# BloodAxe/segmentation-networks-benchmark

Measured on AMD Instinct MI355X. Metric: images/sec/GPU (fwd+bwd) ZF_UNET 224x224 bs=32; 1/2/4/8-GPU scaling, higher is better.
Workload: dtype bf16; 1 GPU; ZF_UNET 224x224 bf16 bs=32/GPU, bce_dice, SGD lr 1e-3, Dropout2d 0.2, train step torch_train.py:180-190 (configs[1]); global_batch=32, parallelism=dp1

## Files before the change

### segmentation-networks-benchmark_amd/csrc/common.h

```cpp
#pragma once
#include <hip/hip_runtime.h>
#include <hip/hip_ext.h>
#include <limits.h>
#include <stdint.h>
#include <stdio.h>
#include <string.h>

#include "../../include/segnb_hip.h"

typedef __attribute__((ext_vector_type(8))) __bf16 bf16x8_t;
typedef __attribute__((ext_vector_type(16))) float f32x16_t;

struct bf16_t {
    unsigned short bits;
};

void segnb_set_error(const char* fmt, ...);

#define SEGNB_CHECK_ARG_AS(who, cond, msg)                           \
    do {                                                             \
        if (!(cond)) {                                               \
            segnb_set_error("%s: bad argument: %s", who, msg);       \
            return SEGNB_E_BADARG;                                   \
        }                                                            \
// ... 34 lines not shown
template <class T>
inline T segnb_plan_keep(T v) {
    static_assert(!(std::is_pointer<T>::value && std::is_class<typename std::remove_pointer<T>::type>::value),
                  "segnb_plan_keep: add an overload that copies this struct into the plan");
    return v;
}
inline const segnb_conv_geom* segnb_plan_keep(const segnb_conv_geom* g) {
    return g ? (const segnb_conv_geom*)segnb_plan_dup(g, sizeof(*g)) : g;
}
inline const segnb_loss_spec* segnb_plan_keep(const segnb_loss_spec* g) {
    return g ? (const segnb_loss_spec*)segnb_plan_dup(g, sizeof(*g)) : g;
}
inline const segnb_bn_reduce_epilogue* segnb_plan_keep(const segnb_bn_reduce_epilogue* g) {
    return g ? (const segnb_bn_reduce_epilogue*)segnb_plan_dup(g, sizeof(*g)) : g;
}
inline const segnb_bn_apply_epilogue* segnb_plan_keep(const segnb_bn_apply_epilogue* g) {
    return g ? (const segnb_bn_apply_epilogue*)segnb_plan_dup(g, sizeof(*g)) : g;
}
inline const segnb_upcat_src* segnb_plan_keep(const segnb_upcat_src* g) {
    return g ? (const segnb_upcat_src*)segnb_plan_dup(g, sizeof(*g)) : g;
}
inline const segnb_operand_tf* segnb_plan_keep(const segnb_operand_tf* g) {
    return g ? (const segnb_operand_tf*)segnb_plan_dup(g, sizeof(*g)) : g;
}
inline const segnb_wgrad_target* segnb_plan_keep(const segnb_wgrad_target* g) {
    return g ? (const segnb_wgrad_target*)segnb_plan_dup(g, sizeof(*g)) : g;
}
inline const segnb_act_epilogue* segnb_plan_keep(const segnb_act_epilogue* g) {
    return g ? (const segnb_act_epilogue*)segnb_plan_dup(g, sizeof(*g)) : g;
}
template <class... P, class... A>
inline void segnb_plan_record_call(const char* name, int (*fn)(P...), A... args) {
    static_assert(sizeof...(P) == sizeof...(A), "argument count");
    std::tuple<P...> kept(segnb_plan_keep((P)args)...);
    segnb_plan_push([fn, kept]() { return std::apply(fn, kept); }, name);
}
extern int g_segnb_census_on;
void segnb_census(const char* name);
#define SEGNB_PLAN_RECORD(fn, ...)                                                           \
    SegnbPlanScope plan_scope__;                                                             \
    if (plan_scope__.top && g_segnb_census_on) segnb_census(#fn);                            \
    if (plan_scope__.top && segnb_plan_recording()) segnb_plan_record_call(#fn, fn, __VA_ARGS__)
void segnb_plan_refuse(const char* why);
#define SEGNB_PLAN_REFUSE(why)                                         \
    SegnbPlanScope plan_scope__;                                       \
    if (plan_scope__.top && g_segnb_census_on) segnb_census(__func__); \
    if (plan_scope__.top && segnb_plan_recording()) segnb_plan_refuse(why)

int segnb_num_cus();
bool segnb_fprop_general_forced();
int segnb_knob_fprop_dma();
int segnb_knob_fprop_dma_cfg();
int segnb_knob_fprop_dma_dbg();
int segnb_knob_fprop_nostats();
int segnb_knob_rw_store_waves();
int segnb_knob_bnreduce_fused();
int segnb_knob_fprop_deepk();
int segnb_knob_fprop_thin();
enum segnb_try_outcome {
    SEGNB_TRY_DECLINED = 0,
    SEGNB_TRY_LAUNCHED,
    SEGNB_TRY_DELIVERED,
};
constexpr int SEGNB_LAUNCH_DECLINED = INT_MIN;
inline int segnb_try_launched(segnb_try_outcome* did, int rc) {
    if (rc == SEGNB_LAUNCH_DECLINED) {
        *did = SEGNB_TRY_DECLINED;
        return 0;
    }
    if (rc == 0) *did = SEGNB_TRY_LAUNCHED;
    return rc;
}
#define SEGNB_HOST_INLINE static inline __attribute__((always_inline))
template <class... K>
int segnb_opt_in_lds(const char* who, int bytes, K... kernels) {
    hipError_t e = hipSuccess;
    (void)(... && ((e = hipFuncSetAttribute(reinterpret_cast<const void*>(kernels), hipFuncAttributeMaxDynamicSharedMemorySize,
                                            bytes)) == hipSuccess));
    if (e != hipSuccess) segnb_set_error("%s hipFuncSetAttribute(%d bytes): %s", who, bytes, hipGetErrorString(e));
    return (int)e;
}
SEGNB_HOST_INLINE long long segnb_nhwc_bytes(long long npix, int ld, int C, int esz) { return ((npix - 1) * ld + C) * esz; }
SEGNB_HOST_INLINE bool segnb_fits_desc(long long bytes, unsigned* out = nullptr) {
    if (out != nullptr) *out = (unsigned)bytes;
    return bytes < (1ll << 31);
}
inline void segnb_kernel_took(segnb_try_outcome did, const char** served, const char* name) {
    if (did != SEGNB_TRY_DECLINED && *served == nullptr) *served = name;
}
template <class Args>
__attribute__((always_inline)) inline bool take_bn_reduce(Args& a, const segnb_conv_geom* g, const segnb_bn_reduce_epilogue* bn) {
    const long long yb = segnb_nhwc_bytes((long long)g->N * g->Ho * g->Wo, bn->ld_y, g->Co, 2);
    if (!segnb_fits_desc(yb)) return false;
    a.bn_y = (const bf16_t*)bn->y;
    a.bn_y_bytes = (unsigned)yb;
    a.bn_ld = bn->ld_y;
    a.bn_coef = bn->coef;
    a.bn_sums = bn->sums;
    a.bn_act = bn->act;
    a.bn_slope = bn->slope;
    return true;
}
template <class Args>
__attribute__((always_inline)) inline void take_act_epilogue(Args& a, const segnb_act_epilogue* ep) {
    a.ep_act = ep != nullptr ? ep->act : -1;
    a.ep_coef = ep != nullptr ? ep->coef : nullptr;
// ... 221 lines not shown
```

### segmentation-networks-benchmark_amd/csrc/fprop_dma.hip

```cpp
#include "common.h"

#include "fprop_dma.h"

#include <mutex>
#include <vector>

#ifndef SEGNB_EXP
#define SEGNB_EXP 0
#endif

namespace {

__device__ unsigned long long g_stamps[3 * 256 * 4];
#define FD_STAMP(role, step, k)                                                                      \
    do {                                                                                            \
        if (DBG && ((a.dbg & 32) || ((a.dbg & 64) && (role) == 0 && (k) == 0)) && blockIdx.x == 0 && lane == 0 &&  \
            (step) < 256)                                                                            \
            g_stamps[((role) * 256 + (step)) * 4 + (k)] = __builtin_amdgcn_s_memtime();             \
    } while (0)

template <int BN_, int R_, int WT_, int CW_M_, bool TALL_ = false, bool MF16_ = true, int NTAP_ = 9, int UP_ = 0>
struct WsCfg {
    static constexpr bool UPD_ = UP_ == 1;
    static constexpr bool UPF = UP_ == 2;
    static_assert(UP_ == 0 || (NTAP_ == 4 && !TALL_ && MF16_), "up-sampled segment forms: 2 x 2 window, 16x16x32 form");
    static constexpr int BN = BN_, R = R_, WT = WT_;
    static constexpr int NTAP = NTAP_, KW = NTAP_ == 9 ? 3 : 2, KH = KW;
    static constexpr bool UPD = UPD_;
    static constexpr int UP = UP_;
    static constexpr int NPL = UPD_ ? 4 : 1;
    static_assert(NTAP_ == 9 || NTAP_ == 4, "3 x 3 or 2 x 2 tap window");
    static_assert(!UPD_ || (NTAP_ == 4 && !TALL_ && MF16_), "plane gather: 2 x 2 window, 16x16x32 form");
    static constexpr bool TALL = TALL_;
    static constexpr bool MF16 = MF16_;
    static constexpr int BM = TALL_ ? 256 : (R_ * WT_ + 16 * CW_M_ - 1) / (16 * CW_M_) * (16 * CW_M_);
    static constexpr int TM16 = BM / CW_M_ / 16, TN16 = BN_ / (4 / CW_M_) / 16;
    static constexpr int NB = 4;
    static constexpr int NT = 512, NCW = 4, NLW = 4;
    static_assert(R * WT <= BM, "tile pixels");
    static constexpr int NRD = TM16 + TN16, NMF = TM16 * TN16;
    static constexpr int rd_before(int q) { return (q * NRD + NMF - 1) / NMF; }
    static constexpr int WAVES_M = CW_M_, WAVES_N = NCW / CW_M_;
    static constexpr int WM = BM / WAVES_M, WN = BN / WAVES_N;
    static constexpr int TM = WM / 32, TN = WN / 32;
    static constexpr int XR = R + KH - 1, XC = WT + 2, NPIX = XR * XC;
    static constexpr int APIECES = (NPIX + 7) / 8;
    static constexpr int A_BYTES = APIECES * 1024;
    static constexpr int NBW = 2, NAW = 2;
    static constexpr int APW = (APIECES + NAW - 1) / NAW;
    static constexpr int A_STEPS = NTAP - 2;
    static constexpr int APS = (APW + A_STEPS - 1) / A_STEPS;
    static constexpr int BPIECES = BN / 8;
    static constexpr int B_STAGE = BN * 128;
    static constexpr int BPW = BPIECES / NBW;
    static constexpr int OUT_ROW = BN * 2 + 16;
    static constexpr int OC = BN / 8;
    static constexpr int MT = NCW * 64;
    static constexpr int RPT = BM / (MT / OC);
    static constexpr int OFF_B = 2 * A_BYTES;
    static constexpr int OFF_STG = OFF_B + NB * B_STAGE;
    static constexpr int OFF_DUMMY = OFF_STG + BM * OUT_ROW;
    static constexpr int OFF_PIX = OFF_DUMMY + 1024;
    static constexpr int OFF_BIAS = OFF_PIX + 4 * BM * 4;
    static constexpr int OFF_SCALE = OFF_BIAS + BN * 4;
    static constexpr int OFF_TICKET = OFF_SCALE + BN * 4;
    static constexpr int SMEM = OFF_TICKET + 16;
    static constexpr int RED_BYTES = MT * 16 * 8;
    static_assert(WM % (MF16_ ? 16 : 32) == 0 && WN % (MF16_ ? 16 : 32) == 0 && WAVES_M * WAVES_N == NCW, "wave tiling");
    static_assert(BPIECES % NBW == 0 && NBW + NAW == NLW, "fetch wave roles");
    static_assert(MT % OC == 0 && MT >= 2 * BN && RPT <= 8 && BM <= MT && BM % (MT / OC) == 0, "store pass / statistics threads");
    static constexpr bool MASK_OK = MF16_ && !TALL_ && BM == 256 && CW_M_ == 4 && SMEM + 2048 <= 160 * 1024;
    static_assert(RED_BYTES <= OFF_STG, "statistics reduction scratch");
    static_assert(SMEM <= 160 * 1024, "LDS");
    static_assert(TM + TN <= 6, "fragment wait statement");
};

template <class C, bool DBG, bool EP = false, bool STATS = true, bool SPLITK = false, bool MASK = false>
__global__ __launch_bounds__(512) void conv_fprop_ws_kernel(const FdArgs a) {
    static_assert(!SPLITK || (!EP && !DBG && C::UP == 0 && C::NTAP == 9), "split K: plain 3 x 3 forward / data gradient");
    static_assert(!MASK || (STATS && !EP && !DBG && !SPLITK && C::MF16 && C::UP == 0 && C::NTAP == 9 && !C::TALL && C::BM == 256 &&
                            C::BN == 64 && C::WAVES_M == 4 && C::SMEM + 2048 <= 160 * 1024),
                  "activation mask: plain 3 x 3 data gradient, 16x16x32 form, 256 x 64 tiles, 2 KB of mask bytes behind the LDS layout");
    constexpr int BN = C::BN, R = C::R, WT = C::WT, BM = C::BM, TM = C::TM, TN = C::TN, XC = C::XC;
    constexpr int NT = C::NT, NB = C::NB, APW = C::APW, APS = C::APS, BPW = C::BPW, OC = C::OC, NLW = C::NLW;
    constexpr int OUT_ROW = C::OUT_ROW, NF = TM + TN;
    constexpr int NTAP = C::NTAP, KW = C::KW;
    constexpr int SM = NTAP & 3;

    extern __shared__ __attribute__((aligned(1024))) unsigned char smem[];
    int* sPix = reinterpret_cast<int*>(smem + C::OFF_PIX);
    float* sBias = reinterpret_cast<float*>(smem + C::OFF_BIAS);
    const unsigned lds0 = (unsigned)(size_t)smem;

    const int tid = threadIdx.x, lane = tid & 63, wave = __builtin_amdgcn_readfirstlane(tid >> 6);
    const int r = lane & 31, h = lane >> 5;
    const bool loader = wave >= C::NCW;
    const int lw = wave - C::NCW;
    const int wm = (wave & 3) / C::WAVES_N, wn = (wave & 3) % C::WAVES_N;

    int L_ = xcd_remap(blockIdx.x, gridDim.x);
    int ks_ = 0, nt_, gq_;
    if (C::TALL && a.ntmajor) {
        gq_ = L_ % a.GM;
        L_ /= a.GM;
        if constexpr (SPLITK) {
            ks_ = L_ % a.KS;
            L_ /= a.KS;
        }
        nt_ = L_;
    } else {
        if constexpr (SPLITK) {
            ks_ = L_ % a.KS;
            L_ /= a.KS;
        }
        nt_ = L_ % a.NTL;
        gq_ = L_ / a.NTL;
    }
    const int ks = ks_;
    const int c_off = SPLITK ? ks * a.NCH : 0;
    const int nt = nt_, gq = gq_;
    int n_base_ = nt * BN, w_row0_ = nt * BN, py_ = 0, px_ = 0;
    if constexpr (C::UPF) {
        const int ph = nt / a.NTLR, ct = nt - ph * a.NTLR;
        n_base_ = ct * BN;
        w_row0_ = ph * a.CoW + ct * BN;
        py_ = ph >> 1;
        px_ = ph & 1;
    }
    const int n_base = n_base_, w_row0 = w_row0_, py = py_, px = px_;

    const i32x4_t rs_x = make_rsrc4(a.x, a.x_bytes);
    const i32x4_t rs_w = make_rsrc4(a.w, a.w_bytes);
    const i32x4_t rs_u = make_rsrc4(a.u != nullptr ? a.u : a.x, a.u != nullptr ? a.u_bytes : a.x_bytes);

    float* sScale = reinterpret_cast<float*>(smem + C::OFF_SCALE);
    for (int c = tid; c < BN; c += NT) {
        const int co = n_base + c;
        const float bv = (a.bias != nullptr && co < a.bias_n) ? a.bias[co] : 0.f;
        float sc = 1.f, sh = bv;
        if constexpr (EP) {
// ... 437 lines not shown
        auto ks_combine = [&](auto&& get, auto&& set) {
            unsigned base = slab0;
            asm volatile("" : "+v"(base));
            if (a.KS == 2) {
                const unsigned other = base + (unsigned)(ks ^ 1) * 65536u;
                static_for<2>([&](auto h_c) {
                    constexpr int h8 = decltype(h_c)::value * 8;
                    f32x4_t o[8];
                    static_for<8>([&](auto q_c) { constexpr int q = decltype(q_c)::value; o[q] = ks_load(other + (h8 + q) * 1024u); });
                    static_for<8>([&](auto q_c) {
                        constexpr int q = decltype(q_c)::value;
                        set(std::integral_constant<int, h8 + q>{}, get(std::integral_constant<int, h8 + q>{}) + o[q]);
                    });
                    asm volatile("s_waitcnt vmcnt(0)" ::: "memory");
                });
            } else {
                static_for<4>([&](auto h_c) {
                    constexpr int h8 = decltype(h_c)::value * 4;
                    f32x4_t v[4][4];
                    static_for<4>([&](auto q_c) {
                        constexpr int q = decltype(q_c)::value;
#pragma unroll
                        for (int k = 0; k < 4; ++k)
                            v[q][k] = ks_load(k != ks ? base + (unsigned)k * 65536u + (h8 + q) * 1024u : OOB);
                    });
                    static_for<4>([&](auto q_c) {
                        constexpr int q = decltype(q_c)::value;
                        const f32x4_t own = get(std::integral_constant<int, h8 + q>{});
#pragma unroll
                        for (int k = 0; k < 4; ++k) v[q][k] = k == ks ? own : v[q][k];
                        set(std::integral_constant<int, h8 + q>{}, (v[q][0] + v[q][1]) + (v[q][2] + v[q][3]));
                    });
                    asm volatile("s_waitcnt vmcnt(0)" ::: "memory");
                });
            }
        };
        if constexpr (MF16) {
            static_assert((TM16 == 4 && TN16 == 4) || (TM16 == 7 && TN16 == 2), "16x16x32 wave tile: 64 x 64 or 112 pixels x 32 channels");
            constexpr int NRD = C::NRD;
            static_assert(NRD + TM16 - 1 <= 15, "counted lgkmcnt");
            bf16x8_t fw[2][TN16], fx[2][TM16];
            auto issue = [&](int q, int set, int wbase, int xbase, int t, int k) {
                if (q == 0) { const int ad = a_rd16[t % KW][0][k] + xbase; FD_READ(fx[set][0], ad); }
                else if (q <= TN16) { const int ad = b_rd16[k][q - 1] + wbase; FD_READ(fw[set][q - 1], ad); }
                else { const int ad = a_rd16[t % KW][q - TN16][k] + xbase; FD_READ(fx[set][q - TN16], ad); }
            };
            int arow[KW];
#pragma unroll
            for (int k = 0; k < KW; ++k) arow[k] = __builtin_amdgcn_readfirstlane(a.dh[KW * k] * XC * 128);
            if (!(DBG && (a.dbg & 4))) {
#pragma unroll
                for (int q = 0; q < NRD; ++q) issue(q, 0, 0, arow[0], 0, 0);
            }
            int tile_no = 0;
            bool pending = false;
            for (; it < a.IT; it += a.GM, ++tile_no) {
                f32x4_t acc[TM16][TN16];
                uint2 prev[C::UPF ? TM16 : 1][C::UPF ? TN16 : 1];
                if constexpr (C::UPF) {
                    const int r16 = lane & 15, g4 = lane >> 4;
                    const int* tab = sPix + (tile_no & 3) * BM;
#pragma unroll
                    for (int i = 0; i < TM16; ++i) {
                        const int opix = tab[wm * C::WM + 16 * i + r16];
#pragma unroll
                        for (int j = 0; j < TN16; ++j) {
                            const int ch = n_base + wn * C::WN + 16 * j + 4 * g4;
                            uint2 v = make_uint2(0u, 0u);
                            if (opix >= 0 && ch < a.Co && !a.no_prev)
                                v = *reinterpret_cast<const uint2*>(a.out + (long long)opix * a.ld_out + ch);
                            prev[i][j] = v;
                        }
                    }
                }
                for (int c = 0; c < a.NCH; ++c, ++cg) {
                    const int a_base = (cg & 1) * C::A_BYTES;
                    const bool drain = pending && c == 0;
                    static_for<NTAP>([&](auto t_c) {
                        constexpr int t = decltype(t_c)::value;
                        constexpr int tn = t == NTAP - 1 ? 0 : t + 1;
                        auto& accr = acc;
                        const int bstage = ((cg * SM + t) & (NB - 1)) * C::B_STAGE;
                        const int bnext = ((cg * SM + t + 1) & (NB - 1)) * C::B_STAGE;
                        const int anext = t == NTAP - 1 ? ((cg + 1) & 1) * C::A_BYTES : a_base;
                        if (wave == 0) FD_STAMP(0, cg * 9 + t, 0);
                        constexpr bool row_tap9 = NTAP == 9 && t >= 1 && t <= C::RPT;
                        bool do_row = false;
                        int krow = t - 1;
                        if constexpr (NTAP == 9) {
                            do_row = drain;
                        } else {
                            const int si = c * NTAP + t;
                            krow = (si - 1) * a.RPS;
                            do_row = pending && si >= 1 && krow < C::RPT;
                        }
                        if constexpr (row_tap9 || NTAP != 9)
                            if (do_row) {
                                row_load(krow, sPix + ((tile_no + 3) & 3) * BM);
                                if constexpr (NTAP != 9)
                                    if (a.RPS == 2) row_load2(krow + 1, sPix + ((tile_no + 3) & 3) * BM);
                            }
                        if (!(SEGNB_EXP & 4) && !(DBG && (a.dbg & 4))) {
                            __builtin_amdgcn_s_setprio(1);
#pragma unroll
                            for (int kk = 0; kk < 2; ++kk) {
                                const int cur = kk, nxt = kk ^ 1;
                                const int wbase = kk == 0 ? bstage : bnext;
                                const int xbase = kk == 0 ? a_base + arow[t / KW] : anext + arow[tn / KW];
// ... 45 lines not shown
                    ks_last = ks_publish([&](auto p_c) { constexpr int p = decltype(p_c)::value; return acc[p / TN16][p % TN16]; });
                    if (ks_last)
                        ks_combine([&](auto p_c) { constexpr int p = decltype(p_c)::value; return acc[p / TN16][p % TN16]; },
                                   [&](auto p_c, const f32x4_t v) { constexpr int p = decltype(p_c)::value; acc[p / TN16][p % TN16] = v; });
                }
                if (!SPLITK || ks_last) {
                const int r16 = lane & 15, g4 = lane >> 4;
                float4 bv[TN16], sv[TN16];
                uint2 mrow[MASK ? TM16 : 1];
                if constexpr (MASK) {
#pragma unroll
                    for (int i = 0; i < TM16; ++i)
                        mrow[i] = *reinterpret_cast<const uint2*>(smem + C::SMEM + (wm * C::WM + 16 * i + r16) * 8);
                }
#pragma unroll
                for (int j = 0; j < TN16; ++j) {
                    if constexpr (!MASK) bv[j] = *reinterpret_cast<const float4*>(sBias + wn * C::WN + 16 * j + 4 * g4);
                    if constexpr (EP) sv[j] = *reinterpret_cast<const float4*>(sScale + wn * C::WN + 16 * j + 4 * g4);
                    else sv[j] = make_float4(1.f, 1.f, 1.f, 1.f);
                }
#pragma unroll
                for (int i = 0; i < TM16; ++i) {
                    const int row = wm * C::WM + 16 * i + r16;
#pragma unroll
                    for (int j = 0; j < TN16; ++j) {
                        const int col = wn * C::WN + 16 * j + 4 * g4;
                        uint2 pk;
                        if constexpr (C::UPF) {
                            const uint2 pv = prev[i][j];
                            const float v0 = acc[i][j][0] + __uint_as_float(pv.x << 16) + bv[j].x;
                            const float v1 = acc[i][j][1] + __uint_as_float(pv.x & 0xffff0000u) + bv[j].y;
                            const float v2 = acc[i][j][2] + __uint_as_float(pv.y << 16) + bv[j].z;
                            const float v3 = acc[i][j][3] + __uint_as_float(pv.y & 0xffff0000u) + bv[j].w;
                            pk.x = pack2bf(fmaxf(v0, v0 * upf_neg), fmaxf(v1, v1 * upf_neg));
                            pk.y = pack2bf(fmaxf(v2, v2 * upf_neg), fmaxf(v3, v3 * upf_neg));
                        } else if constexpr (MASK) {
                            const unsigned mb = (j < 2 ? mrow[i].x : mrow[i].y) >> (8 * ((2 * j + (g4 >> 1)) & 3) + 4 * (g4 & 1));
                            const unsigned g01 = pack2bf(acc[i][j][0], acc[i][j][1]);
                            const unsigned g23 = pack2bf(acc[i][j][2], acc[i][j][3]);
                            const float g0 = __uint_as_float(g01 << 16), g1 = __uint_as_float(g01 & 0xffff0000u);
                            const float g2 = __uint_as_float(g23 << 16), g3 = __uint_as_float(g23 & 0xffff0000u);
                            pk.x = pack2bf((mb & 1u) ? g0 : g0 * mask_neg, (mb & 2u) ? g1 : g1 * mask_neg);
                            pk.y = pack2bf((mb & 4u) ? g2 : g2 * mask_neg, (mb & 8u) ? g3 : g3 * mask_neg);
                        } else {
                        pk.x = pack2bf(ep(acc[i][j][0], sv[j].x, bv[j].x), ep(acc[i][j][1], sv[j].y, bv[j].y));
                        pk.y = pack2bf(ep(acc[i][j][2], sv[j].z, bv[j].z), ep(acc[i][j][3], sv[j].w, bv[j].w));
                        }
                        *reinterpret_cast<uint2*>(sOut + row * OUT_ROW + col * 2) = pk;
                    }
                }
                }
                pending = !SPLITK || ks_last;
            }
            tile_no_out = tile_no;
            pending_out = pending;
        } else {
            static_assert(MF16 || NTAP == 9, "the 32x32x16 form serves the 3 x 3 window only (fragment sets cycle with 36 slices)");

            bf16x8_t fr[3][NF];
            if (!(DBG && (a.dbg & 4))) {
    #pragma unroll
                for (int kk = 0; kk < 2; ++kk) {
    #pragma unroll
                    for (int j = 0; j < TN; ++j) {
                        const int ad = b_rd[j] ^ (kk << 5);
                        FD_READ(fr[kk][j], ad);
                    }
    #pragma unroll
                    for (int i = 0; i < TM; ++i) {
                        const int ad = a_rd[0][i] ^ (kk << 5);
                        FD_READ(fr[kk][TN + i], ad);
                    }
                }
            }
            int tile_no = 0;
            bool pending = false;
            for (; it < a.IT; it += a.GM, ++tile_no) {
                f32x16_t acc[TM][TN];
                for (int c = 0; c < a.NCH; ++c, ++cg) {
                    const int a_base = (cg & 1) * C::A_BYTES;
                    const bool drain = pending && c == 0;
                    static_for<9>([&](auto t_c) {
                        constexpr int t = decltype(t_c)::value;
                        constexpr int tn = t == 8 ? 0 : t + 1;
                        auto& accr = acc;
                        const int bstage = ((cg + t) & (NB - 1)) * C::B_STAGE;
                        const int bnext = ((cg + t + 1) & (NB - 1)) * C::B_STAGE;
                        const int anext = t == 8 ? ((cg + 1) & 1) * C::A_BYTES : a_base;
                        if (wave == 0) FD_STAMP(0, cg * 9 + t, 0);
                        constexpr bool row_tap = t >= 1 && t <= C::RPT;
                        if constexpr (row_tap)
                            if (drain) row_load(t - 1, sPix + ((tile_no + 3) & 3) * BM);
                        if (!(SEGNB_EXP & 4) && !(DBG && (a.dbg & 4))) {
                            __builtin_amdgcn_s_setprio(1);
    #pragma unroll
                            for (int kk = 0; kk < 4; ++kk) {
                                const int set_cur = (4 * t + kk) % 3, set_new = (4 * t + kk + 2) % 3;
                                int ad[NF];
                                if (kk < 2) {
    #pragma unroll
                                    for (int j = 0; j < TN; ++j) ad[j] = (b_rd[j] + bstage) ^ ((kk + 2) << 5);
    #pragma unroll
                                    for (int i = 0; i < TM; ++i) ad[TN + i] = (a_rd[t][i] + a_base) ^ ((kk + 2) << 5);
                                } else {
    #pragma unroll
                                    for (int j = 0; j < TN; ++j) ad[j] = (b_rd[j] + bnext) ^ ((kk - 2) << 5);
// ... 121 lines not shown
    static std::mutex mu;
    static std::vector<Ent> ents;
    int dev = 0;
    if (hipGetDevice(&dev) != hipSuccess) return -1;
    std::lock_guard<std::mutex> lock(mu);
    Ent* e = nullptr;
    for (auto& it : ents)
        if (it.dev == dev && it.stream == stream) e = &it;
    const bool grow = e == nullptr || slab_bytes > e->cap || ntiles > e->ncnt;
    if (grow) {
        hipStreamCaptureStatus cs = hipStreamCaptureStatusNone;
        if (hipStreamIsCapturing(stream, &cs) != hipSuccess || cs != hipStreamCaptureStatusNone) return -1;
        if (e == nullptr) {
            ents.push_back(Ent{dev, stream, nullptr, 0, nullptr, 0});
            e = &ents.back();
        }
        if (slab_bytes > e->cap) {
            float* p = nullptr;
            if (hipMalloc(&p, slab_bytes) != hipSuccess) return -1;
            e->slab = p;
            e->cap = slab_bytes;
        }
        if (ntiles > e->ncnt) {
            const int want = ntiles < 1024 ? 1024 : ntiles;
            int* c = nullptr;
            if (hipMalloc(&c, (size_t)want * sizeof(int)) != hipSuccess) return -1;
            if (hipMemsetAsync(c, 0, (size_t)want * sizeof(int), stream) != hipSuccess) return -1;
            e->cnt = c;
            e->ncnt = want;
        }
    }
    *slab = e->slab;
    *cnt = e->cnt;
    return 0;
}

template <class C>
int ksplit_factor(const FdArgs& a, int it_total, int ntl, int nch) {
    if (!C::TALL || !segnb_knob_fprop_ksplit()) return 1;
    if (a.ep_act >= 0 || a.dbg || a.up_out != nullptr) return 1;
    const long long tiles = (long long)it_total * ntl;
    int cus = segnb_knob_conv_cus();
    if (a.stats == nullptr) cus /= 2;
    int ks = 1;
    if (tiles * 2 <= cus && nch % 2 == 0 && nch / 2 >= 2) ks = 2;
    if (tiles * 4 <= cus && nch % 4 == 0 && nch / 4 >= 2) ks = 4;
    const int forced = segnb_knob_fprop_ksplit();
    if (forced > 1 && nch % forced == 0 && nch / forced >= 2 && (forced == 2 || forced == 4)) ks = forced;
    if (tiles * ks * 65536ll >= (1ll << 31)) return 1;
    return ks;
}

template <class C>
int launch_ws(FdArgs& a, hipStream_t stream) {
    if (a.bn_y != nullptr && !C::MASK_OK) return SEGNB_LAUNCH_DECLINED;
    static const int attr_rc = [] {
        int rc = segnb_opt_in_lds("fprop_ws", C::SMEM, conv_fprop_ws_kernel<C, false>, conv_fprop_ws_kernel<C, true>,
                                  conv_fprop_ws_kernel<C, false, true, false>, conv_fprop_ws_kernel<C, false, false, false>);
        if constexpr (C::MASK_OK) {
            if (rc == 0) rc = segnb_opt_in_lds("fprop_ws", C::SMEM + 2048, conv_fprop_ws_kernel<C, false, false, true, false, true>);
        }
        if constexpr (C::TALL) {
            if (rc == 0)
                rc = segnb_opt_in_lds("fprop_ws", C::SMEM, conv_fprop_ws_kernel<C, false, false, true, true>,
                                      conv_fprop_ws_kernel<C, false, false, false, true>);
        }
        return rc;
    }();
    if (attr_rc) return attr_rc;
    a.HB = (a.H + C::R - 1) / C::R;
    a.WB = (a.W + C::WT - 1) / C::WT;
    a.IT = a.N * a.HB * a.WB;
    if (C::TALL) {
        if (a.W > C::WT || a.Hi != a.H || a.Wi != a.W) return SEGNB_LAUNCH_DECLINED;
        a.IT = (a.N * (a.H + 1) + C::R - 1) / C::R;
    }
    a.NTL = (a.Co + C::BN - 1) / C::BN;
    a.NCH = a.Ci / 64;
    a.KS = 1;
    a.ntmajor = C::TALL ? 1 : 0;
    if constexpr (C::TALL) {
        const int ks = ksplit_factor<C>(a, a.IT, a.NTL, a.NCH);
        if (ks > 1 && ksplit_workspace(stream, (size_t)a.IT * a.NTL * ks * 65536, a.IT * a.NTL, &a.ks_slab, &a.ks_cnt) == 0) {
            a.KS = ks;
            a.NCH /= ks;
            a.GM = a.IT;
            a.ks_slab_bytes = (unsigned)((size_t)a.IT * a.NTL * ks * 65536);
            const dim3 grid(a.IT * a.NTL * ks);
            if (a.stats != nullptr || !segnb_knob_fprop_nostats())
                hipLaunchKernelGGL((conv_fprop_ws_kernel<C, false, false, true, true>), grid, dim3(C::NT), C::SMEM, stream, a);
            else
                hipLaunchKernelGGL((conv_fprop_ws_kernel<C, false, false, false, true>), grid, dim3(C::NT), C::SMEM, stream, a);
            return 0;
        }
    }
    int gm = segnb_knob_conv_cus() / a.NTL;
    if (gm < 1) gm = 1;
    if (gm > a.IT) gm = a.IT;
    a.GM = gm;
    if (a.bn_y != nullptr) {
        if constexpr (C::MASK_OK) {
            hipLaunchKernelGGL((conv_fprop_ws_kernel<C, false, false, true, false, true>), dim3(a.GM * a.NTL), dim3(C::NT), C::SMEM + 2048,
                               stream, a);
            return 0;
        } else {
            return SEGNB_LAUNCH_DECLINED;
        }
    }
    if (a.ep_act >= 0)
        hipLaunchKernelGGL((conv_fprop_ws_kernel<C, false, true, false>), dim3(a.GM * a.NTL), dim3(C::NT), C::SMEM, stream, a);
    else if (a.stats == nullptr && !a.dbg && segnb_knob_fprop_nostats())
        hipLaunchKernelGGL((conv_fprop_ws_kernel<C, false, false, false>), dim3(a.GM * a.NTL), dim3(C::NT), C::SMEM, stream, a);
    else if (a.dbg)
        hipLaunchKernelGGL((conv_fprop_ws_kernel<C, true>), dim3(a.GM * a.NTL), dim3(C::NT), C::SMEM, stream, a);
    else
        hipLaunchKernelGGL((conv_fprop_ws_kernel<C, false>), dim3(a.GM * a.NTL), dim3(C::NT), C::SMEM, stream, a);
    return 0;
}

using WsCfg14 = WsCfg<64, 14, 14, 2, false, true>;

bool ws14_serves(const FdArgs& a) {
    return a.H % 14 == 0 && a.W % 14 == 0 && a.W <= 56 && a.Co > 32 && a.bn_y == nullptr && a.ep_act < 0 && !a.dbg &&
           a.up_out == nullptr && segnb_knob_fprop_mf16();
}

int launch_ws14(FdArgs& a, hipStream_t stream) {
    using C = WsCfg14;
    static const int attr_rc = segnb_opt_in_lds("fprop_ws", C::SMEM, conv_fprop_ws_kernel<C, false>, conv_fprop_ws_kernel<C, false, false, false>);
    if (attr_rc) return attr_rc;
    a.HB = a.H / C::R;
    a.WB = a.W / C::WT;
    a.IT = a.N * a.HB * a.WB;
    a.NTL = (a.Co + C::BN - 1) / C::BN;
    a.NCH = a.Ci / 64;
    a.KS = 1;
    a.ntmajor = 0;
    int gm = segnb_knob_conv_cus() / a.NTL;
    if (gm < 1) gm = 1;
    if (gm > a.IT) gm = a.IT;
    a.GM = gm;
    if (g_segnb_census_on) segnb_census("tile:ws14");
    if (a.stats == nullptr && segnb_knob_fprop_nostats())
        hipLaunchKernelGGL((conv_fprop_ws_kernel<C, false, false, false>), dim3(a.GM * a.NTL), dim3(C::NT), C::SMEM, stream, a);
    else
        hipLaunchKernelGGL((conv_fprop_ws_kernel<C, false>), dim3(a.GM * a.NTL), dim3(C::NT), C::SMEM, stream, a);
    return 0;
}

template <class C>
int launch_ws_upd(FdArgs& a, hipStream_t stream) {
    static const int attr_rc = segnb_opt_in_lds("fprop_ws", C::SMEM, conv_fprop_ws_kernel<C, false, false, false>);
    if (attr_rc) return attr_rc;
    a.HB = (a.H + C::R - 1) / C::R;
    a.WB = (a.W + C::WT - 1) / C::WT;
    a.IT = a.N * a.HB * a.WB;
    a.NTL = (a.Co + C::BN - 1) / C::BN;
    a.P32 = a.Ci == 32;
    a.NCHP = a.P32 ? 1 : a.Ci / 64;
    a.NCH = a.P32 ? 2 : 4 * a.NCHP;
    a.RPS = a.NCH * C::NTAP - 1 < C::RPT ? 2 : 1;
    if ((a.NCH * C::NTAP - 1) * a.RPS < C::RPT) return SEGNB_LAUNCH_DECLINED;
    int gm = segnb_knob_conv_cus() / a.NTL;
    if (gm < 1) gm = 1;
    if (gm > a.IT) gm = a.IT;
    a.GM = gm;
    hipLaunchKernelGGL((conv_fprop_ws_kernel<C, false, false, false>), dim3(a.GM * a.NTL), dim3(C::NT), C::SMEM, stream, a);
    return 0;
}

template <class C>
int launch_ws_upf(FdArgs& a, hipStream_t stream) {
    static const int attr_rc = segnb_opt_in_lds("fprop_ws", C::SMEM, conv_fprop_ws_kernel<C, false, false, true>);
    if (attr_rc) return attr_rc;
    a.HB = (a.H + C::R - 1) / C::R;
    a.WB = (a.W + C::WT - 1) / C::WT;
    a.IT = a.N * a.HB * a.WB;
    a.NTLR = (a.Co + C::BN - 1) / C::BN;
    a.NTL = 4 * a.NTLR;
    a.NCH = a.Ci / 64;
    a.NCHP = a.NCH;
    a.P32 = 0;
    a.RPS = a.NCH * C::NTAP - 1 < C::RPT ? 2 : 1;
    if ((a.NCH * C::NTAP - 1) * a.RPS < C::RPT) return SEGNB_LAUNCH_DECLINED;
    int gm = segnb_knob_conv_cus() / a.NTL;
    if (gm < 1) gm = 1;
    if (gm > a.IT) gm = a.IT;
    a.GM = gm;
    hipLaunchKernelGGL((conv_fprop_ws_kernel<C, false, false, true>), dim3(a.GM * a.NTL), dim3(C::NT), C::SMEM, stream, a);
    return 0;
}

bool upd_geometry(const segnb_conv_geom* g) {
    if (g->ntaps != 16 || g->in_step != 2 || !whole_output(g) || g->Hi != 2 * g->Ho || g->Wi != 2 * g->Wo) return false;
    if ((g->Ci % 64 != 0 && g->Ci != 32) || g->Co <= 32 || g->Wo < 12) return false;
// ... 215 lines not shown
```

### segmentation-networks-benchmark_amd/csrc/runtime.hip

```cpp
#include <stdarg.h>
#include <stdlib.h>

#include "common.h"

static thread_local char g_err[512] = "";

void segnb_set_error(const char* fmt, ...) {
    va_list ap;
    va_start(ap, fmt);
    vsnprintf(g_err, sizeof(g_err), fmt, ap);
    va_end(ap);
}

int segnb_num_cus() {
    static int cus = 0;
    if (cus > 0) return cus;
    int dev = 0;
    hipDeviceProp_t prop;
    if (hipGetDevice(&dev) != hipSuccess || hipGetDeviceProperties(&prop, dev) != hipSuccess) return 256;
    cus = prop.multiProcessorCount > 0 ? prop.multiProcessorCount : 256;
    return cus;
}

extern "C" const char* segnb_last_error(void) { return g_err; }
// ... 258 lines not shown
int segnb_knob_fprop_mf16() {
    if (g_fprop_mf16 == -2) {
        const char* e = getenv("SEGNB_FPROP_MF16");
        g_fprop_mf16 = (e != nullptr && e[0] == '0') ? 0 : 1;
    }
    return g_fprop_mf16;
}
static int g_fprop_upd = -2;
int segnb_knob_fprop_upd() {
    if (g_fprop_upd == -2) {
        const char* e = getenv("SEGNB_FPROP_UPD");
        g_fprop_upd = (e != nullptr && e[0] == '0') ? 0 : 1;
    }
    return g_fprop_upd;
}
static int g_fprop_mask = -2;
int segnb_knob_fprop_mask() {
    if (g_fprop_mask == -2) {
        const char* e = getenv("SEGNB_FPROP_MASK");
        g_fprop_mask = (e != nullptr && e[0] == '0') ? 0 : 1;
    }
    return g_fprop_mask;
}
static int g_fprop_drop = -2;
int segnb_knob_fprop_drop() {
    if (g_fprop_drop == -2) {
        const char* e = getenv("SEGNB_FPROP_DROP");
        g_fprop_drop = (e != nullptr && e[0] == '0') ? 0 : 1;
    }
    return g_fprop_drop;
}
static int g_fprop_nostats = 1;
int segnb_knob_fprop_nostats() { return g_fprop_nostats; }
static int g_rw_store_waves = 4;
int segnb_knob_rw_store_waves() { return g_rw_store_waves; }
static int g_bnreduce_fused = -2;
int segnb_knob_bnreduce_fused() {
    if (g_bnreduce_fused == -2) {
        const char* e = getenv("SEGNB_BNREDUCE_FUSED");
        g_bnreduce_fused = (e != nullptr && e[0] == '0') ? 0 : 1;
    }
    return g_bnreduce_fused;
}
static int g_fprop_ksplit = -2;
int segnb_knob_fprop_ksplit() {
    if (g_fprop_ksplit == -2) {
        const char* e = getenv("SEGNB_FPROP_KSPLIT");
        g_fprop_ksplit = e != nullptr ? atoi(e) : 1;
    }
    return g_fprop_ksplit;
}
static int g_fprop_dma_dbg = 0;
int segnb_knob_fprop_dma_dbg() { return g_fprop_dma_dbg; }
extern "C" int segnb_wg_cu_share(int pct) {
    SEGNB_PLAN_RECORD(segnb_wg_cu_share, pct);
    g_wg_cu_pct = pct < 0 ? 0 : (pct > 100 ? 100 : pct);
    return 0;
}

static thread_local segnb_wgrad_target g_wg_target;
static thread_local bool g_wg_target_armed = false;
extern "C" int segnb_wgrad_target_arm(const segnb_wgrad_target* t) {
    SEGNB_PLAN_RECORD(segnb_wgrad_target_arm, t);
    SEGNB_CHECK_ARG(t != nullptr && t->gw != nullptr, "NULL target");
    SEGNB_CHECK_ARG(t->ntaps >= 1 && t->ntaps <= SEGNB_MAX_TAPS && t->Ci > 0 && t->Co > 0 && t->s_in >= t->ntaps && t->ci_off >= 0 &&
                        t->s_out >= (long long)(t->ci_off + t->Ci) * t->s_in, "bad target layout");
    for (int i = 0; i < t->ntaps; ++i) SEGNB_CHECK_ARG(t->kpos[i] >= 0 && t->kpos[i] < t->s_in, "bad kernel position");
    g_wg_target = *t;
    g_wg_target_armed = true;
    return 0;
}
const segnb_wgrad_target* segnb_take_wgrad_target() {
    if (!g_wg_target_armed) return nullptr;
    g_wg_target_armed = false;
    return &g_wg_target;
}

extern "C" int segnb_tune(const char* key, int value) {
    SEGNB_PLAN_REFUSE("segnb_tune inside a recorded plan");
    SEGNB_CHECK_ARG(key != nullptr, "NULL key");
    if (strcmp(key, "fprop_dma") == 0) {
        g_fprop_dma = value ? 1 : 0;
        return 0;
    }
    if (strcmp(key, "fprop_dma_cfg") == 0) {
        g_fprop_dma_cfg = value < 0 ? -1 : value;
        return 0;
    }
    if (strcmp(key, "fprop_roll") == 0) {
        g_fprop_roll = value < 0 ? 0 : value;
        return 0;
    }
    if (strcmp(key, "pack_blocks") == 0) {
        g_pack_blocks = value < 0 ? 0 : value;
        return 0;
    }
    if (strcmp(key, "wgrad_roll") == 0) {
        g_wgrad_roll = value ? 1 : 0;
        return 0;
    }
    if (strcmp(key, "wgrad_c8roll") == 0) {
        g_wgrad_c8roll = value ? 1 : 0;
        return 0;
    }
    if (strcmp(key, "fprop_rw") == 0) {
        g_fprop_rw = value ? 1 : 0;
// ... 2 lines not shown
    if (strcmp(key, "conv_cu_pct") == 0) {
        g_conv_cu_pct = value < 1 ? 1 : (value > 100 ? 100 : value);
        return 0;
    }
    if (strcmp(key, "plan_profile") == 0) {
        if (value == 2) plan_profile_dump();
        else g_plan_profile = value;
        return 0;
    }
    if (strcmp(key, "wg_cu_pct") == 0) {
        g_wg_cu_pct = value < 0 ? 0 : (value > 100 ? 100 : value);
        return 0;
    }
    if (strcmp(key, "fprop_drop") == 0) {
        g_fprop_drop = value ? 1 : 0;
        return 0;
    }
    if (strcmp(key, "fprop_mask") == 0) {
        g_fprop_mask = value ? 1 : 0;
        return 0;
    }
    if (strcmp(key, "fprop_nostats") == 0) {
        g_fprop_nostats = value ? 1 : 0;
        return 0;
    }
    if (strcmp(key, "rw_store_waves") == 0) {
        g_rw_store_waves = value == 2 ? 2 : (value == 8 ? 8 : 4);
        return 0;
    }
    if (strcmp(key, "bnreduce_fused") == 0) {
        g_bnreduce_fused = value ? 1 : 0;
        return 0;
    }
    if (strcmp(key, "fprop_deepk") == 0) {
        g_fprop_deepk = value ? 1 : 0;
        return 0;
    }
    if (strcmp(key, "fprop_thin") == 0) {
        g_fprop_thin = value ? 1 : 0;
        return 0;
    }
    if (strcmp(key, "fprop_mf16") == 0) {
        g_fprop_mf16 = value ? 1 : 0;
        return 0;
    }
    if (strcmp(key, "call_census") == 0) {
        g_segnb_census_on = value ? 1 : 0;
        return 0;
    }
    if (strcmp(key, "fprop_ksplit") == 0) {
        g_fprop_ksplit = value < 0 ? 0 : value;
        return 0;
    }
    if (strcmp(key, "fprop_dma_dbg") == 0) {
        g_fprop_dma_dbg = value;
        return 0;
    }
    segnb_set_error("segnb_tune: unknown key '%s'", key);
    return SEGNB_E_BADARG;
}

extern "C" int segnb_debug_stamps(unsigned long long* host_dst) {
    SEGNB_CHECK_ARG(host_dst != nullptr, "NULL destination");
    return segnb_fprop_dma_read_stamps(host_dst);
}
```

Baseline: 6969 images/s.

## Interleave previous tile's output stores and BN statistics into MFMA gaps

Adds an EPI variant of the warp-specialized conv forward kernel that spreads the previous tile's row stores and batch-norm statistic accumulation across the MFMA issue slots of the next tile's first taps, instead of running them as a separate epilogue pass. It is enabled by default for the 14x14 and 16x16 tile configurations with 16x16x32 MFMA and 3x3 windows. The aim is to hide store and statistics latency behind matrix work. The cost is extra register pressure and more complex scheduling, and the interleaving may slow the MFMA stream.

Result: faster. 7082 images/s, median of 6 (+1.6%).

```diff
diff --git a/segmentation-networks-benchmark_amd/csrc/common.h b/segmentation-networks-benchmark_amd/csrc/common.h
--- a/segmentation-networks-benchmark_amd/csrc/common.h
+++ b/segmentation-networks-benchmark_amd/csrc/common.h
@@ -110,6 +110,7 @@
 int segnb_knob_fprop_dma();
 int segnb_knob_fprop_dma_cfg();
 int segnb_knob_fprop_dma_dbg();
+int segnb_knob_fprop_dma_epi();
 int segnb_knob_fprop_nostats();
 int segnb_knob_rw_store_waves();
 int segnb_knob_bnreduce_fused();
diff --git a/segmentation-networks-benchmark_amd/csrc/fprop_dma.hip b/segmentation-networks-benchmark_amd/csrc/fprop_dma.hip
--- a/segmentation-networks-benchmark_amd/csrc/fprop_dma.hip
+++ b/segmentation-networks-benchmark_amd/csrc/fprop_dma.hip
@@ -75,6 +75,15 @@
     static_assert(TM + TN <= 6, "fragment wait statement");
 };
 
+template <class C_>
+struct WsEpi : C_ {
+    static constexpr bool EPI = true;
+};
+template <class C, class = void>
+struct ws_epi_of : std::false_type {};
+template <class C>
+struct ws_epi_of<C, std::enable_if_t<C::EPI>> : std::true_type {};
+
 template <class C, bool DBG, bool EP = false, bool STATS = true, bool SPLITK = false, bool MASK = false>
 __global__ __launch_bounds__(512) void conv_fprop_ws_kernel(const FdArgs a) {
     static_assert(!SPLITK || (!EP && !DBG && C::UP == 0 && C::NTAP == 9), "split K: plain 3 x 3 forward / data gradient");
@@ -86,6 +95,8 @@
     constexpr int OUT_ROW = C::OUT_ROW, NF = TM + TN;
     constexpr int NTAP = C::NTAP, KW = C::KW;
     constexpr int SM = NTAP & 3;
+    constexpr bool EPI = ws_epi_of<C>::value;
+    static_assert(!EPI || (C::MF16 && !SPLITK && !EP && C::UP == 0 && C::NTAP == 9), "store rows in the MFMA gaps: 16x16x32 form, 3 x 3 window, whole-K tiles");
 
     extern __shared__ __attribute__((aligned(1024))) unsigned char smem[];
     int* sPix = reinterpret_cast<int*>(smem + C::OFF_PIX);
@@ -629,8 +640,151 @@
 #pragma unroll
                 for (int q = 0; q < NRD; ++q) issue(q, 0, 0, arow[0], 0, 0);
             }
+            constexpr int RSTEPS = STATS ? 10 : 2;
+            constexpr int SLOT0 = (TM16 - 1) * TN16;
+            static_assert(!EPI || (NTAP == 9 && RSTEPS <= 2 * C::NMF - SLOT0), "a store row fits the gaps of a 3 x 3 window's tap");
+            auto epi_tap = [&](auto t_c, auto rows_c, f32x4_t (&accr)[TM16][TN16], bool first_chunk, int tile_no)
+                               __attribute__((always_inline)) {
+                constexpr int t = decltype(t_c)::value, ROWS = decltype(rows_c)::value;
+                constexpr int tn = t == NTAP - 1 ? 0 : t + 1;
+                const int a_base = (cg & 1) * C::A_BYTES;
+                const int bstage = ((cg * SM + t) & (NB - 1)) * C::B_STAGE;
+                const int bnext = ((cg * SM + t + 1) & (NB - 1)) * C::B_STAGE;
+                const int anext = t == NTAP - 1 ? ((cg + 1) & 1) * C::A_BYTES : a_base;
+                if (wave == 0) FD_STAMP(0, cg * 9 + t, 0);
+                if constexpr (ROWS == 1) row_load(t - 1, sPix + ((tile_no + 3) & 3) * BM);
+                unsigned voff = OOB;
+                float rm = 0.f;
+                auto row_step = [&](int k) __attribute__((always_inline)) {
+                    int& pix = row_pix;
+                    u32x4_t& v = row_v;
+                    if (k == 0) {
+                        if (DBG && (a.dbg & (4 | 16))) asm volatile("s_waitcnt lgkmcnt(0)" ::: "memory");
+                        asm volatile("" : "+v"(pix), "+v"(v));
+                        const bool ok = cok && pix >= 0;
+                        voff = ok ? (unsigned)pix * (unsigned)a.ld_out * 2u + (unsigned)(n_base + cc * 8) * 2u : OOB;
+                        rm = ok ? 1.f : 0.f;
+                        asm volatile("" : "+v"(voff), "+v"(rm));
+                    } else if (k == 1) {
+                        asm volatile("" : "+v"(voff), "+v"(v) : : "memory");
+                        if (!(DBG && (a.dbg & 8))) __builtin_amdgcn_raw_buffer_store_b128(v, rs_out, (int)voff, 0, 0);
+                        asm volatile("" ::: "memory");
+                    } else if constexpr (STATS) {
+                        const int e = k - 2;
+                        if constexpr (MASK) asm volatile("" : "+v"(v), "+v"(s1[e]));
+                        else asm volatile("" : "+v"(v), "+v"(s1[e]), "+v"(s2[e]));
+                        const unsigned w = e < 2 ? v.x : e < 4 ? v.y : e < 6 ? v.z : v.w;
+                        const float f = __uint_as_float((e & 1) ? (w & 0xffff0000u) : (w << 16));
+                        const float fm = f * rm;
+                        s1[e] += fm;
+                        if constexpr (!MASK) s2[e] += fm * fm;
+                        if constexpr (MASK) asm volatile("" : "+v"(s1[e]));
+                        else asm volatile("" : "+v"(s1[e]), "+v"(s2[e]));
+                    }
+                };
+                if (!(DBG && (a.dbg & 4))) {
+                    __builtin_amdgcn_s_setprio(1);
+#pragma unroll
+                    for (int kk = 0; kk < 2; ++kk) {
+                        const int cur = kk, nxt = kk ^ 1;
+                        const int wbase = kk == 0 ? bstage : bnext;
+                        const int xbase = kk == 0 ? a_base + arow[t / KW] : anext + arow[tn / KW];
+                        ws_wait_xw<TM16 - 1>(fx[cur][0], fw[cur]);
+#pragma unroll
+                        for (int i = 0; i < TM16; ++i) {
+                            static_for<TM16 - 1>([&](auto k_c) {
+                                constexpr int k = decltype(k_c)::value + 1;
+                                if (i == k) ws_wait1<TM16 - 1 - k + C::rd_before(k * TN16)>(fx[cur][k]);
+                            });
+#pragma unroll
+                            for (int j = 0; j < TN16; ++j) {
+                                const int q = i * TN16 + j;
+                                if (C::rd_before(q + 1) > C::rd_before(q) && !(DBG && (a.dbg & 16))) {
+                                    if (kk == 0) issue(C::rd_before(q), nxt, wbase, xbase, t, 1);
+                                    else issue(C::rd_before(q), nxt, wbase, xbase, tn, 0);
+                                }
+                                const int s = kk * C::NMF + q - SLOT0;
+                                if (!(SEGNB_EXP & 256) && s >= 0 && s < ROWS * RSTEPS) row_step(s);
+                                if (t == 0 && kk == 0 && first_chunk)
+                                    FD_MFMA16_0(accr[i][j], fw[cur][j], fx[cur][i]);
+                                else
+                                    FD_MFMA16(accr[i][j], fw[cur][j], fx[cur][i]);
+                            }
+                        }
+                    }
+                    __builtin_amdgcn_s_setprio(0);
+                    if (SEGNB_EXP & 256) {
+#pragma unroll
+                        for (int s = 0; s < ROWS * RSTEPS; ++s) row_step(s);
+                    }
+                } else {
+#pragma unroll
+                    for (int s = 0; s < ROWS * RSTEPS; ++s) row_step(s);
+                }
+                if (wave == 0) FD_STAMP(0, cg * 9 + t, 1);
+                if (wave == 0) FD_STAMP(0, cg * 9 + t, 2);
+                raw_barrier();
+                if (wave == 0) FD_STAMP(0, cg * 9 + t, 3);
+            };
             int tile_no = 0;
             bool pending = false;
+            if constexpr (EPI) {
+                auto tile_body = [&](auto pend_c) __attribute__((always_inline)) {
+                    constexpr int PEND = decltype(pend_c)::value;
+                    f32x4_t acc[TM16][TN16];
+                    static_for<NTAP>([&](auto t_c) {
+                        constexpr int t = decltype(t_c)::value;
+                        epi_tap(t_c, std::integral_constant<int, (PEND == 1 && t >= 1 && t <= C::RPT) ? 1 : 0>{}, acc, true, tile_no);
+                    });
+                    ++cg;
+                    for (int c = 1; c < a.NCH; ++c, ++cg)
+                        static_for<NTAP>([&](auto t_c) { epi_tap(t_c, std::integral_constant<int, 0>{}, acc, false, tile_no); });
+                    ws_wait_xw<0>(fx[0][0], fw[0]);
+#pragma unroll
+                    for (int i = 1; i < TM16; ++i) ws_wait1<0>(fx[0][i]);
+                    asm volatile("s_nop 7\n\ts_nop 7\n\ts_nop 7" ::);
+                    const int r16 = lane & 15, g4 = lane >> 4;
+                    float4 bv[TN16];
+                    uint2 mrow[MASK ? TM16 : 1];
+                    if constexpr (MASK) {
+#pragma unroll
+                        for (int i = 0; i < TM16; ++i)
+                            mrow[i] = *reinterpret_cast<const uint2*>(smem + C::SMEM + (wm * C::WM + 16 * i + r16) * 8);
+                    } else {
+#pragma unroll
+                        for (int j = 0; j < TN16; ++j) bv[j] = *reinterpret_cast<const float4*>(sBias + wn * C::WN + 16 * j + 4 * g4);
+                    }
+#pragma unroll
+                    for (int i = 0; i < TM16; ++i) {
+                        const int row = wm * C::WM + 16 * i + r16;
+#pragma unroll
+                        for (int j = 0; j < TN16; ++j) {
+                            const int col = wn * C::WN + 16 * j + 4 * g4;
+                            uint2 pk;
+                            if constexpr (MASK) {
+                                const unsigned mb = (j < 2 ? mrow[i].x : mrow[i].y) >> (8 * ((2 * j + (g4 >> 1)) & 3) + 4 * (g4 & 1));
+                                const unsigned g01 = pack2bf(acc[i][j][0], acc[i][j][1]);
+                                const unsigned g23 = pack2bf(acc[i][j][2], acc[i][j][3]);
+                                const float g0 = __uint_as_float(g01 << 16), g1 = __uint_as_float(g01 & 0xffff0000u);
+                                const float g2 = __uint_as_float(g23 << 16), g3 = __uint_as_float(g23 & 0xffff0000u);
+                                pk.x = pack2bf((mb & 1u) ? g0 : g0 * mask_neg, (mb & 2u) ? g1 : g1 * mask_neg);
+                                pk.y = pack2bf((mb & 4u) ? g2 : g2 * mask_neg, (mb & 8u) ? g3 : g3 * mask_neg);
+                            } else {
+                                pk.x = pack2bf(acc[i][j][0] + bv[j].x, acc[i][j][1] + bv[j].y);
+                                pk.y = pack2bf(acc[i][j][2] + bv[j].z, acc[i][j][3] + bv[j].w);
+                            }
+                            *reinterpret_cast<uint2*>(sOut + row * OUT_ROW + col * 2) = pk;
+                        }
+                    }
+                    pending = true;
+                };
+                if (it < a.IT) {
+                    tile_body(std::integral_constant<int, 0>{});
+                    it += a.GM;
+                    ++tile_no;
+                }
+                for (; it < a.IT; it += a.GM, ++tile_no) tile_body(std::integral_constant<int, 1>{});
+            } else {
             for (; it < a.IT; it += a.GM, ++tile_no) {
                 f32x4_t acc[TM16][TN16];
                 uint2 prev[C::UPF ? TM16 : 1][C::UPF ? TN16 : 1];
@@ -782,6 +936,7 @@
                 }
                 pending = !SPLITK || ks_last;
             }
+            }
             tile_no_out = tile_no;
             pending_out = pending;
         } else {
@@ -1009,6 +1164,18 @@
 }
 
 template <class C>
+constexpr bool ws_has_epi() {
+    return C::MF16 && !C::TALL && C::BN == 64 && C::NTAP == 9 && ((C::R == 14 && C::WT == 14) || (C::R == 16 && C::WT == 16));
+}
+bool ws_epi_selected(bool by_default) {
+    const int k = segnb_knob_fprop_dma_epi();
+    const bool on = k < 0 ? by_default : k != 0;
+    if (on && g_segnb_census_on) segnb_census("epi:1");
+    return on;
+}
+constexpr bool WS_EPI_DEFAULT = true;
+
+template <class C>
 int launch_ws(FdArgs& a, hipStream_t stream) {
     if (a.bn_y != nullptr && !C::MASK_OK) return SEGNB_LAUNCH_DECLINED;
     static const int attr_rc = [] {
@@ -1021,6 +1188,15 @@
             if (rc == 0)
                 rc = segnb_opt_in_lds("fprop_ws", C::SMEM, conv_fprop_ws_kernel<C, false, false, true, true>,
                                       conv_fprop_ws_kernel<C, false, false, false, true>);
+        }
+        if constexpr (ws_has_epi<C>()) {
+            using CE = WsEpi<C>;
+            if (rc == 0)
+                rc = segnb_opt_in_lds("fprop_ws", C::SMEM, conv_fprop_ws_kernel<CE, false>, conv_fprop_ws_kernel<CE, true>,
+                                      conv_fprop_ws_kernel<CE, false, false, false>);
+            if constexpr (C::MASK_OK) {
+                if (rc == 0) rc = segnb_opt_in_lds("fprop_ws", C::SMEM + 2048, conv_fprop_ws_kernel<CE, false, false, true, false, true>);
+            }
         }
         return rc;
     }();
@@ -1055,6 +1231,24 @@
     if (gm < 1) gm = 1;
     if (gm > a.IT) gm = a.IT;
     a.GM = gm;
+    if constexpr (ws_has_epi<C>()) {
+        if (a.ep_act < 0 && ws_epi_selected(WS_EPI_DEFAULT)) {
+            using CE = WsEpi<C>;
+            const dim3 grid(a.GM * a.NTL), block(C::NT);
+            if (a.bn_y != nullptr) {
+                if constexpr (C::MASK_OK)
+                    hipLaunchKernelGGL((conv_fprop_ws_kernel<CE, false, false, true, false, true>), grid, block, C::SMEM + 2048, stream, a);
+                else
+                    return SEGNB_LAUNCH_DECLINED;
+            } else if (a.stats == nullptr && !a.dbg && segnb_knob_fprop_nostats())
+                hipLaunchKernelGGL((conv_fprop_ws_kernel<CE, false, false, false>), grid, block, C::SMEM, stream, a);
+            else if (a.dbg)
+                hipLaunchKernelGGL((conv_fprop_ws_kernel<CE, true>), grid, block, C::SMEM, stream, a);
+            else
+                hipLaunchKernelGGL((conv_fprop_ws_kernel<CE, false>), grid, block, C::SMEM, stream, a);
+            return 0;
+        }
+    }
     if (a.bn_y != nullptr) {
         if constexpr (C::MASK_OK) {
             hipLaunchKernelGGL((conv_fprop_ws_kernel<C, false, false, true, false, true>), dim3(a.GM * a.NTL), dim3(C::NT), C::SMEM + 2048,
@@ -1084,7 +1278,9 @@
 
 int launch_ws14(FdArgs& a, hipStream_t stream) {
     using C = WsCfg14;
-    static const int attr_rc = segnb_opt_in_lds("fprop_ws", C::SMEM, conv_fprop_ws_kernel<C, false>, conv_fprop_ws_kernel<C, false, false, false>);
+    using CE = WsEpi<C>;
+    static const int attr_rc = segnb_opt_in_lds("fprop_ws", C::SMEM, conv_fprop_ws_kernel<C, false>, conv_fprop_ws_kernel<C, false, false, false>,
+                                                conv_fprop_ws_kernel<CE, false>, conv_fprop_ws_kernel<CE, false, false, false>);
     if (attr_rc) return attr_rc;
     a.HB = a.H / C::R;
     a.WB = a.W / C::WT;
@@ -1098,6 +1294,13 @@
     if (gm > a.IT) gm = a.IT;
     a.GM = gm;
     if (g_segnb_census_on) segnb_census("tile:ws14");
+    if (ws_epi_selected(WS_EPI_DEFAULT)) {
+        if (a.stats == nullptr && segnb_knob_fprop_nostats())
+            hipLaunchKernelGGL((conv_fprop_ws_kernel<CE, false, false, false>), dim3(a.GM * a.NTL), dim3(C::NT), C::SMEM, stream, a);
+        else
+            hipLaunchKernelGGL((conv_fprop_ws_kernel<CE, false>), dim3(a.GM * a.NTL), dim3(C::NT), C::SMEM, stream, a);
+        return 0;
+    }
     if (a.stats == nullptr && segnb_knob_fprop_nostats())
         hipLaunchKernelGGL((conv_fprop_ws_kernel<C, false, false, false>), dim3(a.GM * a.NTL), dim3(C::NT), C::SMEM, stream, a);
     else
diff --git a/segmentation-networks-benchmark_amd/csrc/runtime.hip b/segmentation-networks-benchmark_amd/csrc/runtime.hip
--- a/segmentation-networks-benchmark_amd/csrc/runtime.hip
+++ b/segmentation-networks-benchmark_amd/csrc/runtime.hip
@@ -334,6 +334,8 @@
 }
 static int g_fprop_dma_dbg = 0;
 int segnb_knob_fprop_dma_dbg() { return g_fprop_dma_dbg; }
+static int g_fprop_dma_epi = -1;
+int segnb_knob_fprop_dma_epi() { return g_fprop_dma_epi; }
 extern "C" int segnb_wg_cu_share(int pct) {
     SEGNB_PLAN_RECORD(segnb_wg_cu_share, pct);
     g_wg_cu_pct = pct < 0 ? 0 : (pct > 100 ? 100 : pct);
@@ -442,6 +444,10 @@
         g_fprop_ksplit = value < 0 ? 0 : value;
         return 0;
     }
+    if (strcmp(key, "fprop_dma_epi") == 0) {
+        g_fprop_dma_epi = value < 0 ? -1 : (value ? 1 : 0);
+        return 0;
+    }
     if (strcmp(key, "fprop_dma_dbg") == 0) {
         g_fprop_dma_dbg = value;
         return 0;
```
